# digitalcytometry/cytospace

Hardware: AMD Instinct MI355X
Metric: cell-to-spot assignments/sec on NxN synthetic cost; bit-exact vs lapjv (higher is better)
Workload: dtype f32

## Files before the change

### cytospace_amd/_lib.py

```python
import ctypes
import os

_HERE = os.path.dirname(os.path.abspath(__file__))
LIB_PATH = os.environ.get("CYTOHIP_LIB") or os.path.join(_HERE, "libcytohip.so")
_lib = None

CYTO_OK = 0
CYTO_ERR_NONFINITE = 2
_EXC = {1: ValueError, 2: ValueError, 3: MemoryError, 7: ValueError, 8: ValueError}
CYTO_ERR_PEER = 9
CYTO_ERR_UNSUPPORTED = 7
CYTO_DTYPE_F32, CYTO_DTYPE_F64, CYTO_DTYPE_U16, CYTO_DTYPE_U8, CYTO_DTYPE_I32, CYTO_DTYPE_I64 = range(6)
CYTO_MTX_ERR_FRACTION, CYTO_MTX_ERR_NONFINITE, CYTO_MTX_ERR_MAGNITUDE, CYTO_MTX_ERR_SQUARE, CYTO_MTX_ERR_IO = range(2, 7)


class CytoHipError(RuntimeError):
    pass


class LapInfo(ctypes.Structure):
    _fields_ = [("ms_colred", ctypes.c_double), ("ms_cache", ctypes.c_double), ("ms_chain", ctypes.c_double),
                ("ms_total", ctypes.c_double)] + \
        [(k, ctypes.c_int64) for k in (
            "scans_colred", "scans_redtransfer", "scans_arr", "scans_aug_init", "scans_aug_relax",
# ... 73 lines not shown
        L.cyto_memcpy_d2h.argtypes = [vp, vp, ctypes.c_size_t, i32]
        L.cyto_device_synchronize.argtypes = [i32]
        for name in ("cyto_lap_f32", "cyto_lap_f64"):
            getattr(L, name).argtypes = [i32, vp, i64, i32, vp, vp, vp, vp, ctypes.POINTER(ctypes.c_double),
                                         ctypes.POINTER(LapInfo), i32, vp]
        for name in ("cyto_lap_f32_opts", "cyto_lap_f64_opts"):
            getattr(L, name).argtypes = [i32, vp, i64, i32, vp, vp, vp, vp, ctypes.POINTER(ctypes.c_double),
                                         ctypes.POINTER(LapInfo), i32, vp, ctypes.POINTER(LapOpts)]
            getattr(L, name).restype = ctypes.c_int
        L.cyto_lap_f32_rowmap.argtypes = [i32, vp, i64, i32, i32, vp, vp, vp, vp, vp, ctypes.POINTER(ctypes.c_double),
                                          ctypes.POINTER(LapInfo), i32, vp, ctypes.POINTER(LapOpts)]
        L.cyto_lap_f32_rowmap.restype = ctypes.c_int
        if hasattr(L, "cyto_wide_embedded_solves"):
            L.cyto_wide_embedded_solves.argtypes = []
            L.cyto_wide_embedded_solves.restype = ctypes.c_longlong
        L.cyto_trim_device_cache.argtypes = [i32]
        L.cyto_trim_device_cache.restype = ctypes.c_int
        dp = ctypes.POINTER(ctypes.c_double)
        L.cyto_lap_f32_from_f64.argtypes = [i32, vp, i64, vp, vp, vp, vp, ctypes.POINTER(ctypes.c_double),
                                            ctypes.POINTER(LapInfo), i32, vp]
        L.cyto_normalize_data.argtypes = [i32, i32, vp, i64, i32, vp, i64, i32]
        L.cyto_standardize.argtypes = [i32, i32, vp, i64, i32, i32, i32, vp, i64, i32, i32, vp]
        L.cyto_cost_pearson.argtypes = [i32, i32, i32, vp, i64, vp, i64, vp, vp, i64, dp, i32, vp]
        L.cyto_transform.argtypes = [i32, i32, i32, vp, i64, i32, i32, i32, vp, i64, i32, i32, vp]
        L.cyto_cost_metric.argtypes = [i32, i32, i32, i32, vp, i64, vp, i64, vp, vp, i64, dp, i32, vp]
        L.cyto_assign_metric.argtypes = [i32, i32, i32, i32, vp, vp, vp, i32, vp, dp, ctypes.POINTER(AssignInfo), i32]
        L.cyto_assign_metric_ex.argtypes = [i32, i32, ctypes.POINTER(Matrix), i32, ctypes.POINTER(Matrix), i32, vp, i32, vp, dp,
                                            ctypes.POINTER(AssignInfo), i32]
        L.cyto_assign_metric_ex.restype = ctypes.c_int
        L.cyto_ctx_create.argtypes = [i32, i32, i32, i32, vp, vp, i32, i32, ctypes.POINTER(vp)]
# ... 65 lines not shown
            getattr(L, name).restype = ctypes.c_int
        _lib = L
    return _lib


def check(status):
    if status == CYTO_OK:
        return
    L = lib()
    msg = L.cyto_strerror(status).decode()
    if status == 5:
        msg += ": " + L.cyto_last_hip_error().decode()
    raise _EXC.get(status, CytoHipError)(f"cytohip status {status}: {msg}")


def wide_embedded_solves():
    return int(lib().cyto_wide_embedded_solves())


def device_count():
    n = ctypes.c_int(0)
    st = lib().cyto_device_count(ctypes.byref(n))
    return n.value if st == CYTO_OK else 0


class DeviceBuffer:

    def __init__(self, nbytes, device_id=0):
        self.device_id = device_id
        self.nbytes = int(nbytes)
# ... 100 lines not shown
```

### cytospace_amd/csrc/lap_jv.hip

```cpp
#include "cyto_common.h"
#include "lap_dev.h"
#include "lap_chain.h"
#include "lap_exact.h"
#include "lap_wide.h"
#include <math.h>
#include <cmath>
#include <type_traits>
#include <vector>
#include <algorithm>
#include <stdlib.h>
#include <stdio.h>
#include <string.h>

namespace cyto {

__global__ void colred_assign(int n, const int32_t *__restrict__ imin, const int32_t *__restrict__ rowsol,
                              int32_t *__restrict__ colsol) {
    const int j = blockIdx.x * blockDim.x + threadIdx.x;
    if (j >= n) return;
    const int i = imin[j];
    colsol[j] = (rowsol[i] == j) ? i : -1;
}

void launch_colred_assign(int n, const int32_t *imin, const int32_t *rowsol, int32_t *colsol, hipStream_t stream) {
// ... 503 lines not shown
        const bool valid = lane < ntail;
        const float raw = valid ? row[c] : 0.0f;
        const float h = valid ? raw - v[c] : INFINITY;
        lmin = fminf(lmin, h);
        one((uint32_t)c, raw, h, valid);
    }
    if (!fail && cnt > KCU) cb_compress(st, lane, 48, cnt, T);
    T_out = T; cnt_out = cnt;
    return !fail && cnt <= KCU && cnt >= 16 && T < INFINITY;
}

template <int U>
__global__ __launch_bounds__(64 * CBW) void build_row_caches_wave(int n, int64_t ld, const float *__restrict__ cost,
                                                                 const float *__restrict__ v, uint32_t *__restrict__ cache_col,
                                                                 float *__restrict__ cache_val, const int32_t *__restrict__ rowmap,
                                                                 const int32_t *__restrict__ same_prev, int stream) {
    __shared__ CbStage stage[CBW];
    const int lane = threadIdx.x & 63, w = __builtin_amdgcn_readfirstlane((int)(threadIdx.x >> 6));
    CbStage &st = stage[w];
    const int gw = (int)blockIdx.x * CBW + w, nw = (int)gridDim.x * CBW;
    const int per = (n + nw - 1) / nw, i_end = min(n, (gw + 1) * per);
    const int nquad = (n + 3) >> 2;
    const __amdgpu_buffer_rsrc_t rv = __builtin_amdgcn_make_buffer_rsrc(const_cast<float *>(v), 0, nquad * 16, 0x00020000);
    float tau_guess = INFINITY, delta = 0.0f;
    for (int i = gw * per; i < i_end; i++) {
        if (same_prev && same_prev[i]) continue;
        const float *__restrict__ row = cost + row_off(rowmap, i, ld);
        const __amdgpu_buffer_rsrc_t rrow = __builtin_amdgcn_make_buffer_rsrc(const_cast<float *>(row), 0, (int)(ld * 4), 0x00020000);
        float tau0 = tau_guess;
        float lmin = INFINITY, dummy = 0.0f, tau = tau0;
        int cnt = 0;
        bool have = false;
        if (stream && (n >> 2) >= 64 * U) {
            have = cb_stream<U>(rrow, rv, row, v, n, lane, tau, cnt, lmin, st);
            if (!have) { tau0 = INFINITY; tau = INFINITY; cnt = 0; }
        } else {
            cnt = cb_sweep<U, true>(rrow, rv, row, v, n, lane, tau0 < INFINITY ? tau0 : -INFINITY, lmin, st);
            have = tau0 < INFINITY && cnt <= KCU && (cnt >= KCU / 2 || cnt >= n);
        }
        if (!have) {
// ... 53 lines not shown
#pragma unroll
        for (int k = 2; k <= 64; k <<= 1) {
#pragma unroll
            for (int j = k >> 1; j > 0; j >>= 1) {
                const uint32_t pk = (uint32_t)__shfl_xor((int)kc, j);
                const float pv = __shfl_xor(kv, j);
                const bool take_min = ((lane & j) == 0) == ((lane & k) == 0);
                const bool sw = take_min ? (pk < kc) : (pk > kc);
                kc = sw ? pk : kc; kv = sw ? pv : kv;
            }
        }
        if (lane == KCU) { kc = COLSENT; kv = tau; }
        cache_col[(int64_t)i * KC + lane] = kc;
        cache_val[(int64_t)i * KC + lane] = kv;
    }
}

#define CHAIN2_FIELDS(P, S)                                                                                             \
    S(int, n) S(int64_t, ld) P(const float, cost) P(float, fws) P(int32_t, iws) P(uint32_t, cache_col) P(float, cache_val)   \
    P(char, misc) P(int32_t, rowgid) P(const int32_t, rowmap) P(float, g_hbest) P(int32_t, g_hstamp)                        \
    S(int, ngroups) S(int, gmode) S(int, auxlds) S(int, aug_start)
#define F_PTR(T, name) T *name;
#define F_GPTR(T, name) __attribute__((address_space(1))) T *name;
#define F_VAL(T, name) T name;
#define F_COPY_PTR(T, name) a.name = (T *)g.name;
#define F_COPY_VAL(T, name) a.name = g.name;
struct Chain2Args { CHAIN2_FIELDS(F_PTR, F_VAL) };
struct Chain2ArgsG { CHAIN2_FIELDS(F_GPTR, F_VAL) };
static_assert(sizeof(Chain2Args) == sizeof(Chain2ArgsG), "mirror layout");
__device__ __forceinline__ Chain2Args load_args(const Chain2Args *__restrict__ batch) {
// ... 1216 lines not shown
    if (o.chain_variant < 0 || o.chain_variant > 3 || o.augmentation < 0 || o.augmentation > 2 || o.inject_exceptions < 0 ||
        o.no_handover < 0 || o.no_handover > 1)
        return CYTO_ERR_BAD_ARG;
    if (o.group_state_global < 0 || o.group_state_global > 1 || o.aux_state_global < 0 || o.aux_state_global > 1) return CYTO_ERR_BAD_ARG;
    if (o.mode < 0 || o.mode > 2 || o.wide_rounds < -1 || o.wide_groups < -1 || o.wide_groups > 32 || o.wide_rebuild < -1 ||
        o.wide_wipe < 0 || o.wide_wipe > 2048 || o.wide_par < -1 || o.wide_par > WIDE_PAR_GMAX) return CYTO_ERR_BAD_ARG;
    if (o.cache_waves < -1 || o.cache_waves > 32 || (o.cache_unroll != 0 && o.cache_unroll != 4 && o.cache_unroll != 8) || o.cache_stream < -1 ||
        o.cache_stream > 1)
        return CYTO_ERR_BAD_ARG;
    if (o.certify < 0 || o.certify > 1 || o.polish < 0 || o.polish > 1) return CYTO_ERR_BAD_ARG;
    if (o.exact < 0 || o.exact > EXACT_SLOTS_MAX || (o.exact && o.polish)) return CYTO_ERR_BAD_ARG;
    for (int r : o.reserved) if (r != 0) return CYTO_ERR_BAD_ARG;
    return CYTO_OK;
}

struct F32Job {
    const float *cost = nullptr; int64_t ld = 0; int cost_on_device = 0;
    const int32_t *rowmap_host = nullptr; int nu = 0;
    int32_t *rowsol = nullptr, *colsol = nullptr; float *u = nullptr, *v = nullptr; double *total = nullptr; cyto_lap_info *info = nullptr;
    int status = CYTO_OK;
    DevBuf slab;
    DevBuf staged, b_fws, b_iws, b_imin, b_pmin, b_parg, b_misc, b_same, b_gid, b_ccol, b_cval, b_ghb, b_ghs, b_lzhb, b_lzhs;
    DevBuf b_rowmap, b_ulist, b_ufirst, b_wide;
    int nused = 0;
    const float *dcost = nullptr; int64_t dld = 0;
    int h_nonfinite = 0, h_ngroups = 0;
    LapStatus h_hand = {};
    Chain2Args c2; LazyArgs la;
    size_t shm_lazy = 0, shm_aug = 0;
    bool alive() const { return status == CYTO_OK; }
    LapStatus *st() const { return b_misc.as<LapStatus>(); }
    const int32_t *rowmap() const { return rowmap_host ? b_rowmap.as<int32_t>() : nullptr; }
    const int32_t *same(int n) const { return (h_ngroups < n && n >= 2) ? b_same.as<int32_t>() : nullptr; }
};

struct F32Plan {
    int n, colblocks, rowblocks, rows_per_block;
    CachePlan cache;
    bool force_l2, lds_variant, lazy, lz_lds_state, lz_cs_lds, no_cs_lds, wide;
    size_t shm_chain, lz_base_shm;
};

int build_caches(const CachePlan &cp, int n, int64_t ld, const float *cost, const int32_t *rowmap, const float *v, uint32_t *cache_col,
                 float *cache_val, const int32_t *same, hipStream_t stream) {
    const int g = std::max(1, std::min((n + CBW - 1) / CBW, cp.waves * cp.cus / CBW));
    if (cp.unroll == 8)
        hipLaunchKernelGGL(build_row_caches_wave<8>, dim3(g), dim3(64 * CBW), 0, stream, n, ld, cost, v, cache_col, cache_val, rowmap, same,
                           cp.stream);
    else
        hipLaunchKernelGGL(build_row_caches_wave<4>, dim3(g), dim3(64 * CBW), 0, stream, n, ld, cost, v, cache_col, cache_val, rowmap, same,
                           cp.stream);
    if (same)
        hipLaunchKernelGGL(replicate_group_caches, dim3(std::max(1, std::min((n + 3) / 4, 2048))), dim3(256), 0, stream, n, same, cache_col,
                           cache_val);
    CYTO_HIP(hipGetLastError());
    return CYTO_OK;
}

template <int CH, bool LDS_STATE>
static int launch_batch(const F32Plan &pl, std::vector<F32Job> &jobs, hipStream_t stream, hipEvent_t ev_cache_done,
                        hipEvent_t ev_arr_done, DevBuf &d_c2, DevBuf &d_la) {
    const int n = pl.n;
    std::vector<int> live;
    for (int b = 0; b < (int)jobs.size(); b++) if (jobs[b].alive()) live.push_back(b);
    const int nl = (int)live.size();
    if (!nl) return CYTO_OK;
// ... 118 lines not shown
    pl.force_l2 = opts.chain_variant != 0;
    pl.no_cs_lds = opts.chain_variant == 3;
    pl.lds_variant = !pl.force_l2 && n <= 13 * per2;
    pl.lazy = opts.augmentation == 2 || !pl.lds_variant || (opts.augmentation == 0 && n > 5120);
    const int npad = (n + 3) & ~3;
    const size_t npad6 = (((size_t)npad * 6) + 15) & ~(size_t)15, npad2 = (((size_t)npad * 2) + 15) & ~(size_t)15;
    const size_t nb24 = (size_t)((((n + 63) / 64) + 511) & ~511) * 8 + (size_t)((n + 63) / 64) * 24 + 16;
    const size_t lds_budget = LDS_DYNAMIC_MAX;
    pl.lz_lds_state = n <= 65535 && !pl.force_l2 && npad6 + nb24 <= lds_budget;
    pl.lz_cs_lds = !pl.lz_lds_state && n <= 65535 && !pl.no_cs_lds && npad2 + nb24 <= lds_budget;
    pl.lz_base_shm = (pl.lz_lds_state ? npad6 : (pl.lz_cs_lds ? npad2 : 0)) + nb24;
    const bool cs_lds_chain = !pl.lds_variant && n <= 65535 && !pl.no_cs_lds;
    pl.shm_chain = pl.lds_variant ? (((size_t)npad * 6 + 15) / 16) * 16 : (cs_lds_chain ? (((size_t)npad * 2 + 15) / 16) * 16 : 16);

    const size_t nT = (size_t)n * sizeof(float), nI = (size_t)n * sizeof(int32_t);
    CYTO_HIP(hipEventRecord(e0, stream));
    for (F32Job &j : jobs) {
        if (!j.cost || j.ld < n) { j.status = CYTO_ERR_BAD_ARG; continue; }
        const int nstored = j.rowmap_host ? j.nu : n;
        std::vector<int32_t> ulist, ufirst;
        if (j.rowmap_host) {
            if (j.nu <= 0) { j.status = CYTO_ERR_BAD_ARG; continue; }
            bool ok = true;
            for (int i = 0; i < n && ok; i++) {
                const int32_t r = j.rowmap_host[i];
                ok = r >= 0 && r < j.nu && (i == 0 || r >= j.rowmap_host[i - 1]);
                if (ok && (i == 0 || r != j.rowmap_host[i - 1])) { ulist.push_back(r); ufirst.push_back(i); }
            }
            if (!ok) { j.status = CYTO_ERR_BAD_ARG; continue; }
            j.nused = (int)ulist.size();
// ... 3 lines not shown
        if (!aligned) {
            j.dld = ((int64_t)n + 3) / 4 * 4;
            if ((rc = j.staged.alloc((size_t)nstored * j.dld * sizeof(float), stream))) return rc;
            CYTO_HIP(hipMemcpy2DAsync(j.staged.p, j.dld * sizeof(float), j.cost, j.ld * sizeof(float), (size_t)n * sizeof(float), nstored,
                                      j.cost_on_device ? hipMemcpyDeviceToDevice : hipMemcpyHostToDevice, stream));
            j.dcost = j.staged.as<float>();
        }
        if (j.rowmap_host) {
            if ((rc = j.b_rowmap.alloc(nI, stream)) || (rc = j.b_ulist.alloc((size_t)j.nused * 4, stream)) || (rc = j.b_ufirst.alloc((size_t)j.nused * 4, stream)))
                return rc;
            CYTO_HIP(hipMemcpyAsync(j.b_rowmap.p, j.rowmap_host, nI, hipMemcpyHostToDevice, stream));
            CYTO_HIP(hipMemcpyAsync(j.b_ulist.p, ulist.data(), (size_t)j.nused * 4, hipMemcpyHostToDevice, stream));
            CYTO_HIP(hipMemcpyAsync(j.b_ufirst.p, ufirst.data(), (size_t)j.nused * 4, hipMemcpyHostToDevice, stream));
            CYTO_HIP(hipStreamSynchronize(stream));
        }
        {
            size_t off = 0;
            auto take = [&](size_t bytes) { const size_t o = off; off += (bytes + 255) & ~(size_t)255; return o; };
            const size_t o_fws = take(6 * nT + 64), o_iws = take(10 * nI + 64), o_imin = take(nI), o_pmin = take((size_t)pl.rowblocks * nT),
                         o_parg = take((size_t)pl.rowblocks * nI), o_misc = take(sizeof(LapStatus)), o_same = take(nI), o_gid = take(nI),
                         o_ccol = take((size_t)n * KC * sizeof(uint32_t)), o_cval = take((size_t)n * KC * sizeof(float));
            if ((rc = j.slab.alloc(off, stream))) return rc;
            char *base = j.slab.as<char>();
            j.b_fws.view(base + o_fws, stream); j.b_iws.view(base + o_iws, stream); j.b_imin.view(base + o_imin, stream);
            j.b_pmin.view(base + o_pmin, stream); j.b_parg.view(base + o_parg, stream); j.b_misc.view(base + o_misc, stream);
            j.b_same.view(base + o_same, stream); j.b_gid.view(base + o_gid, stream); j.b_ccol.view(base + o_ccol, stream);
            j.b_cval.view(base + o_cval, stream);
        }
        float *d_v = j.b_fws.as<float>();
        int32_t *d_rowsol = j.b_iws.as<int32_t>(), *d_colsol = d_rowsol + n, *d_matches = d_rowsol + 2 * (size_t)n;
        CYTO_HIP(hipMemsetAsync(j.b_misc.p, 0, sizeof(LapStatus), stream));
        CYTO_HIP(hipMemsetAsync(d_rowsol, 0xFF, nI, stream));
        CYTO_HIP(hipMemsetAsync(d_matches, 0, nI, stream));
        {
            const int nrows = j.rowmap_host ? j.nused : n;
            const int rpb = j.rowmap_host ? (nrows + pl.rowblocks - 1) / pl.rowblocks : pl.rows_per_block;
            const int rblocks = j.rowmap_host ? (nrows + rpb - 1) / rpb : pl.rowblocks;
            hipLaunchKernelGGL(colred_partial<float>, dim3(pl.colblocks, rblocks), dim3(256), 0, stream, n, j.dld, j.dcost, rpb,
                               j.b_pmin.as<float>(), j.b_parg.as<int32_t>(), &j.st()->nonfinite, nrows,
                               j.rowmap_host ? j.b_ulist.as<int32_t>() : (const int32_t *)nullptr,
                               j.rowmap_host ? j.b_ufirst.as<int32_t>() : (const int32_t *)nullptr);
            hipLaunchKernelGGL(colred_finish<float>, dim3((n + 255) / 256), dim3(256), 0, stream, n, rblocks, j.b_pmin.as<float>(),
                               j.b_parg.as<int32_t>(), d_v, j.b_imin.as<int32_t>(), d_rowsol, d_matches);
        }
        launch_colred_assign(n, j.b_imin.as<int32_t>(), d_rowsol, d_colsol, stream);
    }
    CYTO_HIP(hipGetLastError());
    CYTO_HIP(hipEventRecord(e1, stream));
    const bool want_groups = n >= 2;
    for (F32Job &j : jobs) {
        if (!j.alive()) continue;
        j.h_ngroups = n;
        if (want_groups) {
            if (j.rowmap_host)
                hipLaunchKernelGGL(rows_same_from_map, dim3((n + 255) / 256), dim3(256), 0, stream, n, j.b_rowmap.as<int32_t>(), j.b_same.as<int32_t>());
            else
                hipLaunchKernelGGL(rows_same_as_prev<float>, dim3(min(n, 2048)), dim3(256), 0, stream, n, j.dld, j.dcost, j.b_same.as<int32_t>());
            hipLaunchKernelGGL(rows_group_ids, dim3(1), dim3(1024), 0, stream, n, j.b_same.as<int32_t>(), j.b_gid.as<int32_t>(),
                               &j.st()->ngroups);
        }
        CYTO_HIP(hipMemcpyAsync(&j.h_nonfinite, &j.st()->nonfinite, sizeof(int), hipMemcpyDeviceToHost, stream));
        if (want_groups) CYTO_HIP(hipMemcpyAsync(&j.h_ngroups, &j.st()->ngroups, sizeof(int), hipMemcpyDeviceToHost, stream));
    }
    CYTO_HIP(hipGetLastError());
    CYTO_HIP(hipStreamSynchronize(stream));
    CYTO_HIP(hipEventRecord(e1b, stream));

    for (F32Job &j : jobs) {
        if (!j.alive()) continue;
        if (j.h_nonfinite) { j.status = CYTO_ERR_NONFINITE; continue; }
        if (pl.wide) continue;
        float *d_v = j.b_fws.as<float>(), *d_u = d_v + n;
        int32_t *d_rowsol = j.b_iws.as<int32_t>(), *d_colsol = d_rowsol + n, *d_free = d_rowsol + 3 * (size_t)n;
        const int ng = j.h_ngroups;
// ... 39 lines not shown
        }
        const size_t base_aug = (((pl.lds_variant ? (size_t)npad * 6 : 0) + (c2.gmode == 1 ? (size_t)ng * 8 : 0) + 15) / 16) * 16;
        c2.auxlds = (!opts.aux_state_global && pl.lds_variant && ng < 65536 && base_aug + (size_t)npad * 6 + 4096 <= 160 * 1024) ? 1 : 0;
        j.shm_aug = base_aug + (c2.auxlds ? (size_t)npad * 6 : 0) + 32;
    }

    DevBuf d_c2, d_la;
    if (pl.wide) {
        const WidePlan wp = {n, opts.wide_rounds < 0 ? 0 : (opts.wide_rounds > 0 ? opts.wide_rounds : 4096 + (long long)n / 4),
                             opts.wide_rebuild, opts.wide_wipe, opts.wide_par, pl.cache};
        std::vector<WideJob> wj;
        for (F32Job &j : jobs)
            if (j.alive())
                wj.push_back({j.dcost, j.dld, j.rowmap(), j.b_fws.as<float>(), j.b_iws.as<int32_t>(), j.b_ccol.as<uint32_t>(),
                              j.b_cval.as<float>(), j.b_misc.as<char>(), j.same(n), j.h_ngroups, &j.b_wide});
        rc = wide_solve_batch(wp, wj, stream, e1c, e1d);
    } else if (opts.chain_variant >= 2) rc = launch_batch<0, false>(pl, jobs, stream, e1c, e1d, d_c2, d_la);
    else if (pl.force_l2 && n <= 5 * per2) rc = launch_batch<5, false>(pl, jobs, stream, e1c, e1d, d_c2, d_la);
    else if (pl.force_l2 && n <= 16 * per2) rc = launch_batch<16, false>(pl, jobs, stream, e1c, e1d, d_c2, d_la);
    else if (pl.force_l2) rc = launch_batch<0, false>(pl, jobs, stream, e1c, e1d, d_c2, d_la);
    else if (n <= 2 * per2) rc = launch_batch<2, true>(pl, jobs, stream, e1c, e1d, d_c2, d_la);
    else if (n <= 5 * per2) rc = launch_batch<5, true>(pl, jobs, stream, e1c, e1d, d_c2, d_la);
    else if (n <= 10 * per2) rc = launch_batch<10, true>(pl, jobs, stream, e1c, e1d, d_c2, d_la);
    else if (n <= 13 * per2) rc = launch_batch<13, true>(pl, jobs, stream, e1c, e1d, d_c2, d_la);
    else if (n <= 16 * per2) rc = launch_batch<16, false>(pl, jobs, stream, e1c, e1d, d_c2, d_la);
    else rc = launch_batch<0, false>(pl, jobs, stream, e1c, e1d, d_c2, d_la);
    if (rc) return rc;
    CYTO_HIP(hipEventRecord(e2, stream));
    CYTO_HIP(hipStreamSynchronize(stream));

// ... 24 lines not shown
            CYTO_HIP(hipMemcpyAsync(h_gap, b_viol.as<double>() + n, sizeof h_gap, hipMemcpyDeviceToHost, stream));
            CYTO_HIP(hipStreamSynchronize(stream));
            if (opts.exact && (rc = exact_repair(ex, n, xv, h_gap[0], g, stream))) return rc;
        }
        if (j.rowsol) CYTO_HIP(hipMemcpy(j.rowsol, d_rowsol, nI, hipMemcpyDeviceToHost));
        if (j.colsol) CYTO_HIP(hipMemcpy(j.colsol, d_rowsol + n, nI, hipMemcpyDeviceToHost));
        if (j.u) CYTO_HIP(hipMemcpy(j.u, d_v + n, nT, hipMemcpyDeviceToHost));
        if (j.v) CYTO_HIP(hipMemcpy(j.v, d_v, nT, hipMemcpyDeviceToHost));
        if (j.total) CYTO_HIP(hipMemcpy(j.total, &j.st()->total, sizeof(double), hipMemcpyDeviceToHost));
        if (j.info) {
            cyto_lap_info *info = j.info;
            memset(info, 0, sizeof *info);
            info->ms_colred = ms_colred; info->ms_cache = ms_cache; info->ms_chain = ms_chain; info->ms_arr = ms_arr; info->ms_aug = ms_aug;
            info->ms_total = info->ms_colred + info->ms_cache + info->ms_chain;
            info_from_counters(info, n, h);
            info->hbm_row_reads = 2 * (int64_t)n + h.counters[C_ROWS_READ];
            info->dense_refreshes = h.counters[C2_DENSE_REFRESH];
            info->aug_scans_skipped = h.counters[C2_AUG_SKIPPED];
            info->aug_dense_scans = h.counters[C2_AUG_DENSE];
            info->aug_sparse_inits = h.counters[C2_AUG_SPARSE_INIT];
            info->aug_handover = (pl.lazy && !pl.wide && h.lazy_done < h.numfree) ? h.lazy_done : -1;
            info->row_groups = j.h_ngroups;
            info->certified = h_gap[0] >= 0.0 ? 1 : 0;
            info->gap_f64 = h_gap[0] >= 0.0 ? h_gap[0] : 0.0; info->gap_max_f64 = h_gap[0] >= 0.0 ? h_gap[1] : 0.0;
            info->gap_rows = h_gap[0] >= 0.0 ? (int64_t)h_gap[2] : 0;
            info->exact_status = ex.status; info->exact_edges = ex.edges; info->exact_free_rows = ex.free_rows;
            info->exact_changed_rows = ex.changed; info->exact_overflow_rows = ex.overflow;
            info->exact_ms_emit = ex.ms_emit; info->exact_ms_repair = ex.ms_repair;
            if (pl.wide) {
                const long long *wc = h.wide, *tm = h.timers;
                info->wide = 1;
// ... 114 lines not shown
    if (n <= 0 || !cost_rows || ld < n || !rowmap || nu <= 0) return CYTO_ERR_BAD_ARG;
    return cyto::lap_solve_f32_one(n, cost_rows, ld, cost_on_device, rowmap, nu, rowsol, colsol, u, v, total, info, device_id,
                                   reinterpret_cast<hipStream_t>(stream), opts ? *opts : cyto::k_default_opts);
}

int cyto_lap_f32_opts(int n, const float *cost, int64_t ld, int cost_on_device, int32_t *rowsol, int32_t *colsol,
                      float *u, float *v, double *total, cyto_lap_info *info, int device_id, void *stream, const cyto_lap_opts *opts) {
    return cyto::lap_solve_f32(n, cost, ld, cost_on_device, rowsol, colsol, u, v, total, info, device_id, reinterpret_cast<hipStream_t>(stream), opts ? *opts : cyto::k_default_opts);
}

int cyto_lap_f64_opts(int n, const double *cost, int64_t ld, int cost_on_device, int32_t *rowsol, int32_t *colsol,
                      double *u, double *v, double *total, cyto_lap_info *info, int device_id, void *stream, const cyto_lap_opts *opts) {
    return cyto::lap_solve_f64(n, cost, ld, cost_on_device, rowsol, colsol, u, v, total, info, device_id, reinterpret_cast<hipStream_t>(stream), opts ? *opts : cyto::k_default_opts);
}

}
```

### cytospace_amd/csrc/lap_wide.h

```cpp
#pragma once
#include "cyto_common.h"
#include <vector>

namespace cyto {

constexpr int WIDE_PAR_GMAX = 64;

struct CachePlan {
    int waves = 8, unroll = 4;
    int stream = 1;
    int cus = 256;
};
int build_caches(const CachePlan &cp, int n, int64_t ld, const float *cost, const int32_t *rowmap, const float *v, uint32_t *cache_col,
                 float *cache_val, const int32_t *same, hipStream_t stream);

struct WideJob {
    const float *cost; int64_t ld;
    const int32_t *rowmap;
    float *fws;
    int32_t *iws;
    uint32_t *cache_col; float *cache_val;
    char *misc;
    const int32_t *same;
    int ngroups;
    DevBuf *state;
};
struct WidePlan {
    int n;
    long long rounds;
    int rebuild, wipe, par;
    CachePlan cache;
};
int wide_solve_batch(const WidePlan &pl, const std::vector<WideJob> &jobs, hipStream_t stream, hipEvent_t ev_cache_done,
                     hipEvent_t ev_arr_done);

}
```

### cytospace_amd/csrc/lap_wide.hip

```cpp
#include "lap_dev.h"
#include "lap_wide.h"
#include <algorithm>
#include <atomic>
#include <chrono>
#include <mutex>
#include <thread>
#include <vector>

namespace cyto {

#define WIDE_FIELDS(P, S)                                                                                                  \
    S(int, n) S(int64_t, ld) P(const float, cost) P(const int32_t, rowmap) P(float, v) P(float, u) P(float, cassign)          \
    P(unsigned long long, label) P(unsigned long long, bid) P(int32_t, rowsol) P(int32_t, colsol) P(int32_t, matches)          \
    P(int32_t, freerows) P(int32_t, act0) P(int32_t, act1) P(int32_t, touched) P(int32_t, slot_j) P(float, slot_p)            \
    P(float, slot_c) P(uint32_t, cache_col) P(float, cache_val) P(char, misc) S(long long, max_rounds)                     \
    P(const int32_t, same_prev) P(int32_t, seg_sync) S(int, aug_seg) S(int, aug_waste) S(int, arr_waste) S(int, seg_quorum)   \
    P(char, sc) S(int, par_groups) P(char, par) P(char, scx) P(float, cache_red) P(const int32_t, inv_off) P(const unsigned long long, inv_ent)
#define WIDE_F_PTR(T, name) T *name;
#define WIDE_F_VAL(T, name) T name;
struct WideArgs { WIDE_FIELDS(WIDE_F_PTR, WIDE_F_VAL) };

constexpr size_t WIDE_SC_BYTES = 2048;

namespace {
// ... 2092 lines not shown

int wide_solve_batch(const WidePlan &pl, const std::vector<WideJob> &jobs, hipStream_t stream, hipEvent_t ev_cache_done,
                     hipEvent_t ev_arr_done) {
    const int n = pl.n, nl = (int)jobs.size();
    if (!nl) return CYTO_OK;
    int rc;
    auto build_caches_of = [&](const int32_t *flags) -> int {
        for (int k = 0; k < nl; k++) {
            if (flags && flags[k] == 0) continue;
            const WideJob &j = jobs[(size_t)k];
            const int r = build_caches(pl.cache, n, j.ld, j.cost, j.rowmap, j.fws, j.cache_col, j.cache_val, j.same, stream);
            if (r) return r;
        }
        return CYTO_OK;
    };
    if ((rc = build_caches_of(nullptr))) return rc;
    CYTO_HIP(hipEventRecord(ev_cache_done, stream));
    struct ParSlot { std::atomic<int> *p = nullptr; ~ParSlot() { if (p) p->store(0); } } par_slot;
    int dev_now = 0;
    (void)hipGetDevice(&dev_now);
    const int device_slot = dev_now >= 0 && dev_now < 64 ? dev_now : 0;
    const size_t nT = (size_t)n * sizeof(float);
    const int embed_knob = CYTO_KNOB("CYTO_AUG_EMBED").set ? CYTO_KNOB("CYTO_AUG_EMBED").value : 1;
    std::vector<WideArgs> h_wa((size_t)nl);
    for (int k = 0; k < nl; k++) {
        const WideJob &j = jobs[(size_t)k];
        const int xcd_cus = std::max(1, pl.cache.cus / 8);
        const bool dup_rows = n >= 2 && (long long)j.ngroups * 5 < (long long)n * 4;
        int parg = nl != 1 ? 0 : (pl.par > 0 ? pl.par : (pl.par < 0 || dup_rows || n < 2048 ? 0 : 16));
        parg = std::min(std::min(parg, WIDE_PAR_GMAX), xcd_cus);
        if (parg == 1) parg = 0;
// ... 120 lines not shown
```

### include/cytohip.h

```cpp
#ifndef CYTOHIP_H
#define CYTOHIP_H

#include <stddef.h>
#include <stdint.h>

#ifdef __cplusplus
extern "C" {
#endif

enum {
    CYTO_OK = 0,
    CYTO_ERR_BAD_ARG = 1,
    CYTO_ERR_NONFINITE = 2,
    CYTO_ERR_NOMEM = 3,
    CYTO_ERR_INTERNAL = 4,
    CYTO_ERR_HIP = 5,
    CYTO_ERR_NO_DEVICE = 6,
    CYTO_ERR_UNSUPPORTED = 7,
    CYTO_ERR_SHAPE = 8,
    CYTO_ERR_PEER = 9
};

const char *cyto_strerror(int status);
const char *cyto_last_hip_error(void);
const char *cyto_version(void);
int cyto_abi_sizes(size_t *lap_info, size_t *lap_opts, size_t *assign_info, size_t *chunk);
long long cyto_wide_embedded_solves(void);

int cyto_device_count(int *count);
int cyto_device_name(int device_id, char *buf, size_t buflen);
int cyto_malloc(void **dptr, size_t bytes, int device_id);
int cyto_free(void *dptr, int device_id);
int cyto_memcpy_h2d(void *dst, const void *src, size_t bytes, int device_id);
int cyto_memcpy_d2h(void *dst, const void *src, size_t bytes, int device_id);
int cyto_memcpy_d2d(void *dst, const void *src, size_t bytes, int device_id);
int cyto_device_synchronize(int device_id);
int cyto_trim_device_cache(int device_id);


typedef struct {
    double ms_colred;
    double ms_cache;
// ... 238 lines not shown
```

Measured before the change: 1.256 million.

## Fuse row-cache candidate collection into column reduction pass to skip second cost read

```diff
diff --git a/cytospace_amd/_lib.py b/cytospace_amd/_lib.py
--- a/cytospace_amd/_lib.py
+++ b/cytospace_amd/_lib.py
@@ -111,6 +111,10 @@
         if hasattr(L, "cyto_wide_embedded_solves"):
             L.cyto_wide_embedded_solves.argtypes = []
             L.cyto_wide_embedded_solves.restype = ctypes.c_longlong
+        for name in ("cyto_fused_cache_solves", "cyto_fused_cache_fallback_rows"):
+            if hasattr(L, name):
+                getattr(L, name).argtypes = []
+                getattr(L, name).restype = ctypes.c_longlong
         L.cyto_trim_device_cache.argtypes = [i32]
         L.cyto_trim_device_cache.restype = ctypes.c_int
         dp = ctypes.POINTER(ctypes.c_double)
@@ -206,6 +210,14 @@
     raise _EXC.get(status, CytoHipError)(f"cytohip status {status}: {msg}")
 
 
+def fused_cache_solves():
+    return int(lib().cyto_fused_cache_solves())
+
+
+def fused_cache_fallback_rows():
+    return int(lib().cyto_fused_cache_fallback_rows())
+
+
 def wide_embedded_solves():
     return int(lib().cyto_wide_embedded_solves())
 
diff --git a/cytospace_amd/csrc/lap_jv.hip b/cytospace_amd/csrc/lap_jv.hip
--- a/cytospace_amd/csrc/lap_jv.hip
+++ b/cytospace_amd/csrc/lap_jv.hip
@@ -4,6 +4,7 @@
 #include "lap_exact.h"
 #include "lap_wide.h"
 #include <math.h>
+#include <atomic>
 #include <cmath>
 #include <type_traits>
 #include <vector>
@@ -541,16 +542,19 @@
 __global__ __launch_bounds__(64 * CBW) void build_row_caches_wave(int n, int64_t ld, const float *__restrict__ cost,
                                                                  const float *__restrict__ v, uint32_t *__restrict__ cache_col,
                                                                  float *__restrict__ cache_val, const int32_t *__restrict__ rowmap,
-                                                                 const int32_t *__restrict__ same_prev, int stream) {
+                                                                 const int32_t *__restrict__ same_prev, int stream,
+                                                                 const int32_t *__restrict__ rowlist, int count) {
     __shared__ CbStage stage[CBW];
     const int lane = threadIdx.x & 63, w = __builtin_amdgcn_readfirstlane((int)(threadIdx.x >> 6));
     CbStage &st = stage[w];
     const int gw = (int)blockIdx.x * CBW + w, nw = (int)gridDim.x * CBW;
-    const int per = (n + nw - 1) / nw, i_end = min(n, (gw + 1) * per);
+    const int nrows = rowlist ? count : n;
+    const int per = (nrows + nw - 1) / nw, i_end = min(nrows, (gw + 1) * per);
     const int nquad = (n + 3) >> 2;
     const __amdgpu_buffer_rsrc_t rv = __builtin_amdgcn_make_buffer_rsrc(const_cast<float *>(v), 0, nquad * 16, 0x00020000);
     float tau_guess = INFINITY, delta = 0.0f;
-    for (int i = gw * per; i < i_end; i++) {
+    for (int ii = gw * per; ii < i_end; ii++) {
+        const int i = rowlist ? __builtin_amdgcn_readfirstlane(rowlist[ii]) : ii;
         if (same_prev && same_prev[i]) continue;
         const float *__restrict__ row = cost + row_off(rowmap, i, ld);
         const __amdgpu_buffer_rsrc_t rrow = __builtin_amdgcn_make_buffer_rsrc(const_cast<float *>(row), 0, (int)(ld * 4), 0x00020000);
@@ -634,6 +638,201 @@
         cache_col[(int64_t)i * KC + lane] = kc;
         cache_val[(int64_t)i * KC + lane] = kv;
     }
+}
+
+constexpr int FUSED_S = 2048;
+constexpr int FUSED_TARGET = 190;
+constexpr int COLRED_CAP = 512;
+struct ColredAppend {
+    const float *w; const float *theta;
+    int32_t *cnt; uint2 *list;
+};
+__global__ __launch_bounds__(256) void colred_partial_append(int n, int64_t ld, const float *__restrict__ cost, int rows_per_block,
+                                                             float *__restrict__ pmin, int32_t *__restrict__ parg,
+                                                             int *__restrict__ nonfinite, int nrows, ColredAppend ap) {
+    constexpr int VW = 4, RU = 4;
+    const int q = blockIdx.x * 256 + threadIdx.x;
+    const int col0 = q * VW, ql = min(q, (n - 1) >> 2);
+    const int r0 = blockIdx.y * rows_per_block;
+    const int r1 = min(nrows, r0 + rows_per_block);
+    const int lane = threadIdx.x & 63;
+    const uint64_t lt = (1ull << lane) - 1ull;
+    float mn[VW], we[VW];
+    int32_t arg[VW];
+    bool bad = false;
+#pragma unroll
+    for (int e = 0; e < VW; e++) { mn[e] = INFINITY; arg[e] = r0; we[e] = col0 + e < n ? ap.w[col0 + e] : 0.0f; }
+    auto row_of = [&](int k) { return min(r0 + k, r1 - 1); };
+    auto load_row = [&](int r) { return *(reinterpret_cast<const float4 *>(cost + (int64_t)r * ld) + ql); };
+    float4 xn[RU]; float thn[RU];
+#pragma unroll
+    for (int u = 0; u < RU; u++) { xn[u] = load_row(row_of(u)); thn[u] = ap.theta[row_of(u)]; }
+    for (int k = 0; r0 + k < r1; k += RU) {
+        float4 x[RU]; float thr[RU]; int rr[RU];
+#pragma unroll
+        for (int u = 0; u < RU; u++) {
+            x[u] = xn[u]; thr[u] = thn[u]; rr[u] = row_of(k + u);
+            asm volatile("" : "+v"(x[u].x), "+v"(x[u].y), "+v"(x[u].z), "+v"(x[u].w), "+v"(thr[u]) :: "memory");
+        }
+#pragma unroll
+        for (int u = 0; u < RU; u++) { xn[u] = load_row(row_of(k + RU + u)); thn[u] = ap.theta[row_of(k + RU + u)]; }
+        uint64_t b[RU][VW]; int tot[RU];
+        int my_tot = 0, my_row = 0;
+#pragma unroll
+        for (int u = 0; u < RU; u++) {
+            tot[u] = 0;
+            const float th = r0 + k + u < r1 ? thr[u] : -INFINITY;
+#pragma unroll
+            for (int e = 0; e < VW; e++) {
+                const float xe = vec_get<float>(x[u], e);
+                if (col0 + e < n) bad |= !__builtin_isfinite(xe);
+                if (xe < mn[e]) { mn[e] = xe; arg[e] = rr[u]; }
+                b[u][e] = __ballot(col0 + e < n && xe - we[e] < th);
+                tot[u] += __popcll(b[u][e]);
+            }
+            if (lane == u) { my_tot = tot[u]; my_row = rr[u]; }
+        }
+        uint32_t old = 0;
+        if (my_tot) old = (uint32_t)atomicAdd(ap.cnt + my_row, my_tot);
+        asm volatile("" : "+v"(old) :: "memory");
+#pragma unroll
+        for (int u = 0; u < RU; u++) {
+            if (!tot[u]) continue;
+            int pos = __builtin_amdgcn_readlane((int)old, u);
+            uint2 *lst = ap.list + (int64_t)rr[u] * COLRED_CAP;
+#pragma unroll
+            for (int e = 0; e < VW; e++) {
+                const int p = pos + __popcll(b[u][e] & lt);
+                if (((b[u][e] >> lane) & 1ull) && (unsigned)p < (unsigned)COLRED_CAP)
+                    lst[p] = make_uint2((uint32_t)(col0 + e), __float_as_uint(vec_get<float>(x[u], e)));
+                pos += __popcll(b[u][e]);
+            }
+        }
+    }
+#pragma unroll
+    for (int e = 0; e < VW; e++) {
+        if (col0 + e < n) {
+            pmin[(int64_t)blockIdx.y * n + col0 + e] = mn[e];
+            parg[(int64_t)blockIdx.y * n + col0 + e] = arg[e];
+        }
+    }
+    if (bad) atomicOr(nonfinite, 1);
+}
+
+
+static int fused_min_kept(int n) {
+    const double c0 = std::min(49.0, std::max(6.0, (double)FUSED_TARGET * FUSED_S / n));
+    return (int)std::min(48.0, std::max(16.0, 0.5 * c0 * n / FUSED_S));
+}
+
+__global__ void fused_w(int n, int nblocks, const float *__restrict__ pmin, float *__restrict__ w) {
+    const int j = blockIdx.x * blockDim.x + threadIdx.x;
+    if (j >= n) return;
+    float mn = pmin[j];
+    for (int b = 1; b < nblocks; b++) mn = fminf(mn, pmin[(int64_t)b * n + j]);
+    w[j] = mn;
+}
+
+__global__ __launch_bounds__(256) void fused_theta(int n, int64_t ld, const float *__restrict__ cost, const float *__restrict__ w,
+                                                   float *__restrict__ theta) {
+    const int lane = threadIdx.x & 63, i = (int)blockIdx.x * 4 + (int)(threadIdx.x >> 6);
+    if (i >= n) return;
+    const float4 *row = reinterpret_cast<const float4 *>(cost + (int64_t)i * ld), *w4 = reinterpret_cast<const float4 *>(w);
+    float m = INFINITY;
+#pragma unroll
+    for (int u = 0; u < FUSED_S / 256; u++) {
+        const float4 x = row[64 * u + lane], y = w4[64 * u + lane];
+        m = fminf(m, fminf(fminf(x.x - y.x, x.y - y.y), fminf(x.z - y.z, x.w - y.w)));
+    }
+    const float srt = cb_sort64(m, lane);
+    const float c0 = fminf(49.0f, fmaxf(6.0f, (float)FUSED_TARGET * (float)FUSED_S / (float)n));
+    const int i0 = (int)(64.0f * (1.0f - __expf(-(c0 + 1.0f) * 0.015625f)));
+    const float th = __shfl(srt, i0);
+    if (lane == 0) theta[i] = th;
+}
+
+__global__ __launch_bounds__(256) void fused_fixup(int n, const float *__restrict__ v, const float *__restrict__ theta,
+                                                   const int32_t *__restrict__ cnt, const uint2 *__restrict__ list,
+                                                   const int32_t *__restrict__ same_prev, uint32_t *__restrict__ cache_col,
+                                                   float *__restrict__ cache_val, int32_t *__restrict__ rowlist, int32_t *__restrict__ nfail,
+                                                   int min_kept) {
+    constexpr int NT = COLRED_CAP / 64;
+    __shared__ uint32_t s_col[4][KC];
+    __shared__ float s_val[4][KC];
+    const int lane = threadIdx.x & 63, w = __builtin_amdgcn_readfirstlane((int)(threadIdx.x >> 6));
+    const int i = (int)blockIdx.x * 4 + w;
+    if (i >= n) return;
+    if (same_prev && same_prev[i]) return;
+    const int c = __builtin_amdgcn_readfirstlane(cnt[i]);
+    const uint64_t lt = (1ull << lane) - 1ull;
+    float tau = theta[i];
+    bool fail = c > COLRED_CAP;
+    int kept = 0;
+    if (!fail) {
+        const int nt = (c + 63) >> 6;
+        uint32_t col[NT]; float raw[NT], h[NT];
+        int below = 0;
+#pragma unroll
+        for (int t = 0; t < NT; t++) {
+            col[t] = 0; raw[t] = 0.0f; h[t] = INFINITY;
+            if (t < nt) {
+                const int k = 64 * t + lane;
+                if (k < c) {
+                    const uint2 e = list[(int64_t)i * COLRED_CAP + k];
+                    col[t] = e.x; raw[t] = __uint_as_float(e.y);
+                    const float hh = raw[t] - v[e.x];
+                    if (hh < tau) h[t] = hh;
+                }
+                below += __popcll(__ballot(h[t] < INFINITY));
+            }
+        }
+        if (below > KCU) {
+            uint32_t key[NT];
+#pragma unroll
+            for (int t = 0; t < NT; t++) key[t] = f2ord(h[t]);
+            uint32_t P = 0;
+            for (int bit = 31; bit >= 0; bit--) {
+                const uint32_t cand = P | (1u << bit);
+                int lower = 0;
+#pragma unroll
+                for (int t = 0; t < NT; t++) if (t < nt) lower += __popcll(__ballot(key[t] < cand));
+                if (lower <= KCU) P = cand;
+            }
+            tau = ord2f(P);
+        }
+#pragma unroll
+        for (int t = 0; t < NT; t++) {
+            if (t < nt) {
+                const bool keep = h[t] < tau;
+                const uint64_t m = __ballot(keep);
+                if (keep) { const int p = kept + __popcll(m & lt); s_col[w][p] = col[t]; s_val[w][p] = raw[t]; }
+                kept += __popcll(m);
+            }
+        }
+        fail = kept < min_kept && n > 16;
+    }
+    if (fail) {
+        if (lane == 0) rowlist[atomicAdd(nfail, 1)] = i;
+        return;
+    }
+    __builtin_amdgcn_fence(__ATOMIC_ACQ_REL, "wavefront");
+    __builtin_amdgcn_wave_barrier();
+    uint32_t kc = lane < kept ? s_col[w][lane] : COLSENT;
+    float kv = lane < kept ? s_val[w][lane] : 0.0f;
+#pragma unroll
+    for (int k = 2; k <= 64; k <<= 1) {
+#pragma unroll
+        for (int j = k >> 1; j > 0; j >>= 1) {
+            const uint32_t pk = (uint32_t)__shfl_xor((int)kc, j);
+            const float pv = __shfl_xor(kv, j);
+            const bool take_min = ((lane & j) == 0) == ((lane & k) == 0);
+            const bool sw = take_min ? (pk < kc) : (pk > kc);
+            kc = sw ? pk : kc; kv = sw ? pv : kv;
+        }
+    }
+    if (lane == KCU) { kc = COLSENT; kv = tau; }
+    cache_col[(int64_t)i * KC + lane] = kc;
+    cache_val[(int64_t)i * KC + lane] = kv;
 }
 
 #define CHAIN2_FIELDS(P, S)                                                                                             \
@@ -1880,6 +2079,8 @@
     return CYTO_OK;
 }
 
+static std::atomic<long long> g_fused_solves{0}, g_fused_fallback_rows{0};
+
 struct F32Job {
     const float *cost = nullptr; int64_t ld = 0; int cost_on_device = 0;
     const int32_t *rowmap_host = nullptr; int nu = 0;
@@ -1891,6 +2092,8 @@
     int nused = 0;
     const float *dcost = nullptr; int64_t dld = 0;
     int h_nonfinite = 0, h_ngroups = 0;
+    bool fused = false; int h_fused_failed = 0;
+    float *f_w = nullptr, *f_theta = nullptr; int32_t *f_cnt = nullptr, *f_rows = nullptr, *f_nfail = nullptr; uint2 *f_list = nullptr;
     LapStatus h_hand = {};
     Chain2Args c2; LazyArgs la;
     size_t shm_lazy = 0, shm_aug = 0;
@@ -1908,14 +2111,15 @@
 };
 
 int build_caches(const CachePlan &cp, int n, int64_t ld, const float *cost, const int32_t *rowmap, const float *v, uint32_t *cache_col,
-                 float *cache_val, const int32_t *same, hipStream_t stream) {
-    const int g = std::max(1, std::min((n + CBW - 1) / CBW, cp.waves * cp.cus / CBW));
-    if (cp.unroll == 8)
+                 float *cache_val, const int32_t *same, hipStream_t stream, const int32_t *rowlist, int count) {
+    const int nrows = rowlist ? count : n;
+    const int g = std::max(1, std::min((nrows + CBW - 1) / CBW, cp.waves * cp.cus / CBW));
+    if (nrows > 0 && cp.unroll == 8)
         hipLaunchKernelGGL(build_row_caches_wave<8>, dim3(g), dim3(64 * CBW), 0, stream, n, ld, cost, v, cache_col, cache_val, rowmap, same,
-                           cp.stream);
-    else
+                           cp.stream, rowlist, count);
+    else if (nrows > 0)
         hipLaunchKernelGGL(build_row_caches_wave<4>, dim3(g), dim3(64 * CBW), 0, stream, n, ld, cost, v, cache_col, cache_val, rowmap, same,
-                           cp.stream);
+                           cp.stream, rowlist, count);
     if (same)
         hipLaunchKernelGGL(replicate_group_caches, dim3(std::max(1, std::min((n + 3) / 4, 2048))), dim3(256), 0, stream, n, same, cache_col,
                            cache_val);
@@ -2064,6 +2268,10 @@
     pl.shm_chain = pl.lds_variant ? (((size_t)npad * 6 + 15) / 16) * 16 : (cs_lds_chain ? (((size_t)npad * 2 + 15) / 16) * 16 : 16);
 
     const size_t nT = (size_t)n * sizeof(float), nI = (size_t)n * sizeof(int32_t);
+    const int fused_knob = CYTO_KNOB("CYTO_CACHE_FUSED").set ? CYTO_KNOB("CYTO_CACHE_FUSED").value : 1;
+    const bool fused_gate = fused_knob != 0 && nb == 1 && pl.wide && !jobs[0].rowmap_host && pl.cache.stream == 1 &&
+                            n >= (fused_knob >= 2 ? FUSED_S : 32768);
+    const int fused_rs = std::min(1024, n / 2);
     CYTO_HIP(hipEventRecord(e0, stream));
     for (F32Job &j : jobs) {
         if (!j.cost || j.ld < n) { j.status = CYTO_ERR_BAD_ARG; continue; }
@@ -2097,18 +2305,29 @@
             CYTO_HIP(hipMemcpyAsync(j.b_ufirst.p, ufirst.data(), (size_t)j.nused * 4, hipMemcpyHostToDevice, stream));
             CYTO_HIP(hipStreamSynchronize(stream));
         }
-        {
+        j.fused = fused_gate;
+        for (;;) {
             size_t off = 0;
             auto take = [&](size_t bytes) { const size_t o = off; off += (bytes + 255) & ~(size_t)255; return o; };
             const size_t o_fws = take(6 * nT + 64), o_iws = take(10 * nI + 64), o_imin = take(nI), o_pmin = take((size_t)pl.rowblocks * nT),
                          o_parg = take((size_t)pl.rowblocks * nI), o_misc = take(sizeof(LapStatus)), o_same = take(nI), o_gid = take(nI),
                          o_ccol = take((size_t)n * KC * sizeof(uint32_t)), o_cval = take((size_t)n * KC * sizeof(float));
-            if ((rc = j.slab.alloc(off, stream))) return rc;
+            const size_t o_fw = j.fused ? take(nT + 16) : 0, o_fth = j.fused ? take(nT) : 0, o_fcnt = j.fused ? take(nI + 256) : 0,
+                         o_frows = j.fused ? take(nI) : 0, o_flist = j.fused ? take((size_t)n * COLRED_CAP * sizeof(uint2)) : 0;
+            rc = j.slab.alloc(off, stream);
+            if (rc == CYTO_ERR_NOMEM && j.fused) { (void)hipGetLastError(); j.fused = false; continue; }
+            if (rc) return rc;
             char *base = j.slab.as<char>();
+            if (j.fused) {
+                j.f_w = reinterpret_cast<float *>(base + o_fw); j.f_theta = reinterpret_cast<float *>(base + o_fth);
+                j.f_cnt = reinterpret_cast<int32_t *>(base + o_fcnt); j.f_nfail = j.f_cnt + n;
+                j.f_rows = reinterpret_cast<int32_t *>(base + o_frows); j.f_list = reinterpret_cast<uint2 *>(base + o_flist);
+            }
             j.b_fws.view(base + o_fws, stream); j.b_iws.view(base + o_iws, stream); j.b_imin.view(base + o_imin, stream);
             j.b_pmin.view(base + o_pmin, stream); j.b_parg.view(base + o_parg, stream); j.b_misc.view(base + o_misc, stream);
             j.b_same.view(base + o_same, stream); j.b_gid.view(base + o_gid, stream); j.b_ccol.view(base + o_ccol, stream);
             j.b_cval.view(base + o_cval, stream);
+            break;
         }
         float *d_v = j.b_fws.as<float>();
         int32_t *d_rowsol = j.b_iws.as<int32_t>(), *d_colsol = d_rowsol + n, *d_matches = d_rowsol + 2 * (size_t)n;
@@ -2119,6 +2338,19 @@
             const int nrows = j.rowmap_host ? j.nused : n;
             const int rpb = j.rowmap_host ? (nrows + pl.rowblocks - 1) / pl.rowblocks : pl.rows_per_block;
             const int rblocks = j.rowmap_host ? (nrows + rpb - 1) / rpb : pl.rowblocks;
+            if (j.fused) {
+                const int srb0 = std::max(1, std::min(pl.rowblocks, (fused_rs + 15) / 16)), srpb = (fused_rs + srb0 - 1) / srb0,
+                          srb = (fused_rs + srpb - 1) / srpb;
+                hipLaunchKernelGGL(colred_partial<float>, dim3(pl.colblocks, srb), dim3(256), 0, stream, n, j.dld, j.dcost, srpb,
+                                   j.b_pmin.as<float>(), j.b_parg.as<int32_t>(), &j.st()->nonfinite, fused_rs, (const int32_t *)nullptr,
+                                   (const int32_t *)nullptr);
+                hipLaunchKernelGGL(fused_w, dim3((n + 255) / 256), dim3(256), 0, stream, n, srb, j.b_pmin.as<float>(), j.f_w);
+                hipLaunchKernelGGL(fused_theta, dim3((n + 3) / 4), dim3(256), 0, stream, n, j.dld, j.dcost, j.f_w, j.f_theta);
+                CYTO_HIP(hipMemsetAsync(j.f_cnt, 0, nI + sizeof(int32_t), stream));
+                const ColredAppend ap = {j.f_w, j.f_theta, j.f_cnt, j.f_list};
+                hipLaunchKernelGGL(colred_partial_append, dim3(pl.colblocks, rblocks), dim3(256), 0, stream, n, j.dld, j.dcost, rpb,
+                                   j.b_pmin.as<float>(), j.b_parg.as<int32_t>(), &j.st()->nonfinite, nrows, ap);
+            } else
             hipLaunchKernelGGL(colred_partial<float>, dim3(pl.colblocks, rblocks), dim3(256), 0, stream, n, j.dld, j.dcost, rpb,
                                j.b_pmin.as<float>(), j.b_parg.as<int32_t>(), &j.st()->nonfinite, nrows,
                                j.rowmap_host ? j.b_ulist.as<int32_t>() : (const int32_t *)nullptr,
@@ -2141,6 +2373,11 @@
                 hipLaunchKernelGGL(rows_same_as_prev<float>, dim3(min(n, 2048)), dim3(256), 0, stream, n, j.dld, j.dcost, j.b_same.as<int32_t>());
             hipLaunchKernelGGL(rows_group_ids, dim3(1), dim3(1024), 0, stream, n, j.b_same.as<int32_t>(), j.b_gid.as<int32_t>(),
                                &j.st()->ngroups);
+        }
+        if (j.fused) {
+            hipLaunchKernelGGL(fused_fixup, dim3((n + 3) / 4), dim3(256), 0, stream, n, j.b_fws.as<float>(), j.f_theta, j.f_cnt, j.f_list,
+                               j.b_same.as<int32_t>(), j.b_ccol.as<uint32_t>(), j.b_cval.as<float>(), j.f_rows, j.f_nfail, fused_min_kept(n));
+            CYTO_HIP(hipMemcpyAsync(&j.h_fused_failed, j.f_nfail, sizeof(int), hipMemcpyDeviceToHost, stream));
         }
         CYTO_HIP(hipMemcpyAsync(&j.h_nonfinite, &j.st()->nonfinite, sizeof(int), hipMemcpyDeviceToHost, stream));
         if (want_groups) CYTO_HIP(hipMemcpyAsync(&j.h_ngroups, &j.st()->ngroups, sizeof(int), hipMemcpyDeviceToHost, stream));
@@ -2210,6 +2447,13 @@
             if (j.alive())
                 wj.push_back({j.dcost, j.dld, j.rowmap(), j.b_fws.as<float>(), j.b_iws.as<int32_t>(), j.b_ccol.as<uint32_t>(),
                               j.b_cval.as<float>(), j.b_misc.as<char>(), j.same(n), j.h_ngroups, &j.b_wide});
+        if (jobs[0].fused && !wj.empty()) {
+            F32Job &j = jobs[0];
+            if (j.h_fused_failed <= n / 8) { wj[0].first_rows = j.f_rows; wj[0].first_count = j.h_fused_failed; }
+            else j.h_fused_failed = n;
+            g_fused_solves.fetch_add(1);
+            g_fused_fallback_rows.fetch_add(j.h_fused_failed);
+        }
         rc = wide_solve_batch(wp, wj, stream, e1c, e1d);
     } else if (opts.chain_variant >= 2) rc = launch_batch<0, false>(pl, jobs, stream, e1c, e1d, d_c2, d_la);
     else if (pl.force_l2 && n <= 5 * per2) rc = launch_batch<5, false>(pl, jobs, stream, e1c, e1d, d_c2, d_la);
@@ -2264,7 +2508,7 @@
             info->ms_colred = ms_colred; info->ms_cache = ms_cache; info->ms_chain = ms_chain; info->ms_arr = ms_arr; info->ms_aug = ms_aug;
             info->ms_total = info->ms_colred + info->ms_cache + info->ms_chain;
             info_from_counters(info, n, h);
-            info->hbm_row_reads = 2 * (int64_t)n + h.counters[C_ROWS_READ];
+            info->hbm_row_reads = (j.fused ? (int64_t)n + fused_rs + j.h_fused_failed : 2 * (int64_t)n) + h.counters[C_ROWS_READ];
             info->dense_refreshes = h.counters[C2_DENSE_REFRESH];
             info->aug_scans_skipped = h.counters[C2_AUG_SKIPPED];
             info->aug_dense_scans = h.counters[C2_AUG_DENSE];
@@ -2409,4 +2653,7 @@
     return cyto::lap_solve_f64(n, cost, ld, cost_on_device, rowsol, colsol, u, v, total, info, device_id, reinterpret_cast<hipStream_t>(stream), opts ? *opts : cyto::k_default_opts);
 }
 
-}
+long long cyto_fused_cache_solves(void) { return cyto::g_fused_solves.load(); }
+long long cyto_fused_cache_fallback_rows(void) { return cyto::g_fused_fallback_rows.load(); }
+
+}
diff --git a/cytospace_amd/csrc/lap_wide.h b/cytospace_amd/csrc/lap_wide.h
--- a/cytospace_amd/csrc/lap_wide.h
+++ b/cytospace_amd/csrc/lap_wide.h
@@ -12,7 +12,7 @@
     int cus = 256;
 };
 int build_caches(const CachePlan &cp, int n, int64_t ld, const float *cost, const int32_t *rowmap, const float *v, uint32_t *cache_col,
-                 float *cache_val, const int32_t *same, hipStream_t stream);
+                 float *cache_val, const int32_t *same, hipStream_t stream, const int32_t *rowlist = nullptr, int count = 0);
 
 struct WideJob {
     const float *cost; int64_t ld;
@@ -24,6 +24,7 @@
     const int32_t *same;
     int ngroups;
     DevBuf *state;
+    const int32_t *first_rows = nullptr; int first_count = -1;
 };
 struct WidePlan {
     int n;
diff --git a/cytospace_amd/csrc/lap_wide.hip b/cytospace_amd/csrc/lap_wide.hip
--- a/cytospace_amd/csrc/lap_wide.hip
+++ b/cytospace_amd/csrc/lap_wide.hip
@@ -2130,7 +2130,11 @@
         }
         return CYTO_OK;
     };
-    if ((rc = build_caches_of(nullptr))) return rc;
+    if (nl == 1 && jobs[0].first_count >= 0) {
+        const WideJob &j = jobs[0];
+        if ((rc = build_caches(pl.cache, n, j.ld, j.cost, j.rowmap, j.fws, j.cache_col, j.cache_val, j.same, stream, j.first_rows, j.first_count)))
+            return rc;
+    } else if ((rc = build_caches_of(nullptr))) return rc;
     CYTO_HIP(hipEventRecord(ev_cache_done, stream));
     struct ParSlot { std::atomic<int> *p = nullptr; ~ParSlot() { if (p) p->store(0); } } par_slot;
     int dev_now = 0;
diff --git a/include/cytohip.h b/include/cytohip.h
--- a/include/cytohip.h
+++ b/include/cytohip.h
@@ -26,6 +26,8 @@
 const char *cyto_version(void);
 int cyto_abi_sizes(size_t *lap_info, size_t *lap_opts, size_t *assign_info, size_t *chunk);
 long long cyto_wide_embedded_solves(void);
+long long cyto_fused_cache_solves(void);
+long long cyto_fused_cache_fallback_rows(void);
 
 int cyto_device_count(int *count);
 int cyto_device_name(int device_id, char *buf, size_t buflen);
```

New measurement: 1.335 million (median of 6 runs). 1.06x the previous value.
